# l90lpa/fv3-jedi-linearmodel

Measured on AMD Instinct MI355X. Metric: column-updates/s per TL+AD dyn step, higher is better.
Workload: dtype f64

## Files before the change

fv3_jedi_linearmodel_amd/csrc/fv3lm_capi.cpp:

```cpp
#include "dynamics.h"
#include <array>
#include <string>

using namespace fv3;

struct fv3lm_handle { Dynamics d; };

static thread_local std::string g_err;
static int fail(const std::string& m) { g_err = m; return 1; }
static int g_live = 0;

extern "C" {

const char* fv3lm_last_error(void) { return g_err.c_str(); }

const char* fv3lm_metric_names(void) {
  return "area,rarea,rarea_c,dx,dy,dxa,dya,dxc,dyc,rdx,rdy,rdxa,rdya,rdxc,rdyc,cosa,sina,rsina,cosa_u,cosa_v,cosa_s,"
         "sina_u,sina_v,rsin_u,rsin_v,rsin2,f0,fC,del6_u,del6_v,divg_u,divg_v,"
         "sin_sg1,sin_sg2,sin_sg3,sin_sg4,sin_sg5,sin_sg6,sin_sg7,sin_sg8,sin_sg9,"
         "cos_sg1,cos_sg2,cos_sg3,cos_sg4,cos_sg5,cos_sg6,cos_sg7,cos_sg8,cos_sg9";
}

int fv3lm_create(fv3lm_handle** out, const fv3lm_dims* dm, const fv3lm_options* opt, const double* const* metrics,
                 double da_min, double da_min_c, const double* phis, const double* ak, const double* bk) {
  if (!out || !dm || !opt || !metrics) return fail("fv3lm_create: null argument");
#ifndef FV3LM_HOST_EMUL
  int ndev = 0;
  if (hipGetDeviceCount(&ndev) != hipSuccess || ndev < 1) return fail("fv3lm_create: no HIP device visible (this library has no CPU fallback)");
#endif
  if (!sticky_error().empty()) {
    if (g_live > 0) return fail("fv3lm_create: an earlier failure of a live handle is pending: " + sticky_error());
    sticky_error().clear();
  }
  fv3lm_handle* h = new fv3lm_handle;
  auto bail = [&](std::string e) { h->d.destroy2(); h->d.destroy(); delete h; sticky_error().clear(); return fail("fv3lm_create: " + e); };
  if (!h->d.init(dm->nx, dm->ny, dm->npz, dm->ntile, dm->face, dm->nq, dm->dt, dm->n_split, dm->k_split, *opt, metrics, da_min,
                 da_min_c, phis, dm->nface, dm->tile_ij0)) return bail(h->d.err);
  if (!sticky_error().empty()) return bail(sticky_error());
  if (!h->d.init2(ak, bk)) return bail(h->d.err);
  if (!sticky_error().empty()) return bail(sticky_error());
  *out = h;
  ++g_live;
  return 0;
}

int fv3lm_destroy(fv3lm_handle* h) {
  if (!h) return 0;
  h->d.destroy2(); h->d.destroy(); delete h;
  if (--g_live <= 0) { g_live = 0; sticky_error().clear(); }
  return 0;
}

static bool find(fv3lm_handle* h, const char* name, Fld& f) {
  if (std::string(name) == "phis") { f = Fld{}; f.t = h->d.hs_dev; f.p = h->d.hs_dev; f.nk = 1; return true; }
  auto it = h->d.F.find(name);
  if (it == h->d.F.end()) { g_err = std::string("unknown field ") + name; return false; }
  f = it->second; return true;
}
int fv3lm_field_levels(fv3lm_handle* h, const char* name) { Fld f; return find(h, name, f) ? f.nk : -1; }
int fv3lm_field_put(fv3lm_handle* h, const char* name, int which, const double* host) {
  Fld f; if (!find(h, name, f)) return 1;
  h2d(h->d.ex, which ? f.p : f.t, host, (size_t)h->d.g.ntile * f.nk * h->d.g.plane * 8);
  return sticky_error().empty() ? 0 : fail(sticky_error());
}
int fv3lm_field_get(fv3lm_handle* h, const char* name, int which, double* host) {
  Fld f; if (!find(h, name, f)) return 1;
  d2h(h->d.ex, host, which ? f.p : f.t, (size_t)h->d.g.ntile * f.nk * h->d.g.plane * 8);
  return sticky_error().empty() ? 0 : fail(sticky_error());
}
static int status(fv3lm_handle* h) {
#ifndef FV3LM_HOST_EMUL
  { const hipError_t e = hipGetLastError();
    if (e != hipSuccess) set_sticky(std::string("HIP kernel launch failed: ") + hipGetErrorString(e)); }
  if (const char* dbg = std::getenv("FV3LM_DEBUG_SYNC")) if (dbg[0] == '1') {
    const hipError_t e = hipStreamSynchronize(h->d.ex.stream);
    if (e != hipSuccess) set_sticky(std::string("HIP stream failed: ") + hipGetErrorString(e));
  }
#endif
  if (!sticky_error().empty()) return fail(sticky_error());
  if (!h->d.err.empty() && h->d.halo_missing) return fail(h->d.err);
  if (h->d.halo_missing) return fail("halo exchange needed before fv3lm_set_exchange provided its table (face mode)");
  if (h->d.tracer_subcycle_error) return fail("tracer_2d: accumulated Courant number > 60: trajectory is not usable");
  if (h->d.nh_overflow()) return fail("non-hydrostatic column solver: reverse-mode tape overflow (internal sizing error)");
  return 0;
}
int fv3lm_set_face_data(fv3lm_handle* h, const double* edge, const double* ecorner) {
  if (!edge || !ecorner) return fail("fv3lm_set_face_data: null argument");
  return h->d.set_face_data(edge, ecorner) ? 0 : fail(h->d.err);
}
int fv3lm_set_rayleigh(fv3lm_handle* h, double tau, double rf_cutoff, const double* c2l) {
  if (!h) return fail("fv3lm_set_rayleigh: null handle");
  if (!h->d.set_rayleigh(tau, rf_cutoff, c2l)) return fail(h->d.err);
  return status(h);
}
int fv3lm_rayleigh_profile(fv3lm_handle* h, double* rf, int* kmax) {
  if (!h || !rf || !kmax) return fail("fv3lm_rayleigh_profile: null argument");
  for (int k = 0; k < h->d.g.npz; ++k) rf[k] = k < (int)h->d.rf_host.size() ? h->d.rf_host[(size_t)k] : 0.;
  *kmax = h->d.rf_kmax;
  return 0;
}
int fv3lm_set_exchange(fv3lm_handle* h, int kind, const int* rows, int nrows) {
  if (!rows && nrows > 0) return fail("fv3lm_set_exchange: null table");
  return h->d.set_exchange(kind, rows, nrows) ? 0 : fail(h->d.err);
}
int fv3lm_set_exchange_remote(fv3lm_handle* h, int kind, int npeers, const int* peers, const int* nsend, const int* send_rows, const int* nrecv,
                              const int* recv_rows) {
  return h->d.set_exchange_remote(kind, npeers, peers, nsend, send_rows, nrecv, recv_rows) ? 0 : fail(h->d.err);
}
int fv3lm_comm_unique_id(const char* rccl_path, void* id128) {
#ifndef FV3LM_HOST_EMUL
  std::string e; Transport& T = transport();
  if (!T.load(rccl_path, e)) return fail(e);
  ncclUniqueId id;
  if (T.pGetUniqueId(&id) != ncclSuccess) return fail("ncclGetUniqueId failed");
  std::memcpy(id128, &id, sizeof id);
  return 0;
#else
  (void)rccl_path; (void)id128; return fail("host emulation has no RCCL; use fv3lm_set_transport_callback");
#endif
}
int fv3lm_comm_init(const char* rccl_path, const void* id128, int nranks, int rank) {
#ifndef FV3LM_HOST_EMUL
  std::string e; Transport& T = transport();
  if (!T.load(rccl_path, e)) return fail(e);
  ncclUniqueId id; std::memcpy(&id, id128, sizeof id);
  if (T.pCommInitRank(&T.comm, nranks, id, rank) != ncclSuccess) return fail("ncclCommInitRank failed");
  T.rank = rank; T.nranks = nranks;
  return 0;
#else
  (void)rccl_path; (void)id128; (void)nranks; (void)rank; return fail("host emulation has no RCCL; use fv3lm_set_transport_callback");
#endif
}
int fv3lm_comm_destroy(void) {
#ifndef FV3LM_HOST_EMUL
  Transport& T = transport();
  if (T.comm && T.pCommDestroy) T.pCommDestroy(T.comm);
  T.comm = nullptr;
#endif
  return 0;
}
int fv3lm_set_allreduce_callback(fv3lm_allreduce_fn fn, void* user) { allreduce_max_hook().cb = fn; allreduce_max_hook().user = user; return 0; }
int fv3lm_set_transport_callback(fv3lm_transport_fn fn, void* user) { transport().cb = fn; transport().user = user; return 0; }
int fv3lm_halo(fv3lm_handle* h, int kind, const char* name0, const char* name1, int mode) {
  if (mode < 0 || mode > 2 || kind < 0 || kind >= H_NKIND) return fail("bad mode or kind");
  Fld f0, f1{};
  auto it = h->d.F.find(name0);
  if (it == h->d.F.end()) return fail(std::string("unknown field ") + name0);
  f0 = it->second;
  if (name1 && name1[0]) { it = h->d.F.find(name1); if (it == h->d.F.end()) return fail(std::string("unknown field ") + name1); f1 = it->second; }
  h->d.halo(mode, kind, f0, f1);
  return status(h);
}
int fv3lm_run_group(fv3lm_handle* h, const char* group, int mode) {
  if (mode < 0 || mode > 2) return fail("bad mode");
  h->d.ex.no_wmask = group && group[0];
  h->d.run_group(h->d.acoustic, group, mode);
  h->d.ex.no_wmask = false;
  return status(h);
}
int fv3lm_dyn_core(fv3lm_handle* h, int mode) {
  if (mode < 0 || mode > 2) return fail("bad mode");
  h->d.dyn_core(mode);
  return status(h);
}
int fv3lm_pressures(fv3lm_handle* h, int mode) { h->d.pressures(mode); return status(h); }
int fv3lm_tracer_2d(fv3lm_handle* h, int mode) {
  if (mode == MODE_AD) h->d.tracer_ad(); else h->d.tracer_fwd(mode);
  return status(h);
}
int fv3lm_traj_slots(fv3lm_handle* h) { return (int)h->d.traj_slot.size(); }
int fv3lm_tracer_nsplt(fv3lm_handle* h) { return h->d.nsplt_max; }
int fv3lm_remap(fv3lm_handle* h, int mode, int last_step) { h->d.each_class([&]() { run_remap(h->d.ex, mode, h->d.remap_args(last_step != 0)); }); return status(h); }
int fv3lm_fv_dynamics(fv3lm_handle* h, int mode) { h->d.fv_dynamics(mode); return status(h); }
int fv3lm_rayleigh(fv3lm_handle* h, int mode) {
  if (mode < 0 || mode > 2) return fail("bad mode");
  h->d.rayleigh(mode);
  return status(h);
}
int fv3lm_step_tl(fv3lm_handle* h) { h->d.step_tl(); return status(h); }
int fv3lm_step_nl(fv3lm_handle* h) { h->d.step_nl(); return status(h); }
int fv3lm_step_ad(fv3lm_handle* h) { h->d.step_ad(); return status(h); }
int fv3lm_traj_to_fv3(fv3lm_handle* h, const double* u, const double* v, const double* t, const double* delp, const double* const* q,
                      const double* w, const double* delz, const double* phis) {
  if (!h->d.traj_to_fv3(u, v, t, delp, q, w, delz, phis)) return fail(h->d.err);
  return status(h);
}
int fv3lm_pert_to_fv3(fv3lm_handle* h, const double* u, const double* v, const double* t, const double* delp, const double* const* q,
                      const double* w, const double* delz) {
  if (!h->d.pert_to_fv3(u, v, t, delp, q, w, delz)) return fail(h->d.err);
  return status(h);
}
int fv3lm_fv3_to_pert(fv3lm_handle* h, double* u, double* v, double* t, double* delp, double* const* q, double* w, double* delz) {
  if (!h->d.fv3_to_pert(u, v, t, delp, q, w, delz)) return fail(h->d.err);
  return status(h);
}
int fv3lm_zero_work_adjoint(fv3lm_handle* h) { h->d.zero_work_adjoint(); return 0; }
int fv3lm_sync(fv3lm_handle* h) { dev_sync(h->d.ex); return status(h); }
long fv3lm_launch_count(fv3lm_handle* h) { return h->d.ex.launches; }
int fv3lm_level_params(fv3lm_handle* h, int k, int* ip, double* rp) {
  if (k < 1 || k > h->d.g.npz) return fail("level out of range");
  const LevelParams& l = h->d.lev_host[k - 1];
  ip[0] = l.hord_mt; ip[1] = l.hord_vt; ip[2] = l.hord_tm; ip[3] = l.hord_dp; ip[4] = l.hord_tr;
  ip[5] = l.nord; ip[6] = l.nord_v; ip[7] = l.nord_w; ip[8] = l.nord_t; ip[9] = l.nord_v_pert;
  rp[0] = l.d2_divg; rp[1] = l.damp_vt; rp[2] = l.damp_w; rp[3] = l.damp_t; rp[4] = l.d_con; rp[5] = l.damp_vt_pert;
  return 0;
}
int fv3lm_set_device(int dev) {
#ifndef FV3LM_HOST_EMUL
  if (hipSetDevice(dev) != hipSuccess) return fail("hipSetDevice failed");
#endif
  (void)dev; return 0;
}
int fv3lm_state_save(fv3lm_handle* h) {
  Dynamics& d = h->d; std::vector<Fld> fs{d.f("u"), d.f("v"), d.f("pt"), d.f("delp")};
  if (d.nh) { fs.push_back(d.f("w")); fs.push_back(d.f("delz")); }
  for (auto& q : d.q) fs.push_back(q);
  if (d.snap.size() != fs.size() * 2) { for (double* p : d.snap) dev_free(p); d.snap.clear(); for (size_t n = 0; n < fs.size() * 2; ++n) d.snap.push_back((double*)dev_alloc(d.n3 * 8)); }
  for (size_t n = 0; n < fs.size(); ++n) { dev_copy(d.ex, d.snap[2 * n], fs[n].t, d.n3 * 8); dev_copy(d.ex, d.snap[2 * n + 1], fs[n].p, d.n3 * 8); }
  return 0;
}
int fv3lm_state_restore(fv3lm_handle* h) {
  Dynamics& d = h->d; std::vector<Fld> fs{d.f("u"), d.f("v"), d.f("pt"), d.f("delp")};
  if (d.nh) { fs.push_back(d.f("w")); fs.push_back(d.f("delz")); }
  for (auto& q : d.q) fs.push_back(q);
  if (d.snap.size() != fs.size() * 2) return fail("fv3lm_state_restore: no snapshot");
  for (size_t n = 0; n < fs.size(); ++n) { dev_copy(d.ex, fs[n].t, d.snap[2 * n], d.n3 * 8); dev_copy(d.ex, fs[n].p, d.snap[2 * n + 1], d.n3 * 8); }
  return 0;
}
int fv3lm_profile_begin(fv3lm_handle* h) { h->d.ex.recs.clear(); h->d.ex.profiling = true; return 0; }
int fv3lm_profile_end(fv3lm_handle* h, char* buf, int buflen) {
  Exec& ex = h->d.ex; ex.profiling = false; dev_sync(ex);
  std::map<std::string, std::array<double, 3>> agg;
  for (ProfRec& r : ex.recs) {
    float ms = 0.f;
#ifndef FV3LM_HOST_EMUL
    (void)hipEventElapsedTime(&ms, r.e0, r.e1); (void)hipEventDestroy(r.e0); (void)hipEventDestroy(r.e1);
#endif
    auto& a = agg[r.name]; a[0] += 1.; a[1] += ms; a[2] += r.bytes;
  }
  ex.recs.clear();
  std::string out;
  for (auto& kv : agg) { char line[256]; std::snprintf(line, sizeof line, "%s %.0f %.6f %.0f\n", kv.first.c_str(), kv.second[0], kv.second[1], kv.second[2]); out += line; }
  if (buf && buflen > 0) { std::strncpy(buf, out.c_str(), buflen - 1); buf[buflen - 1] = 0; }
  return (int)out.size() + 1;
}
#ifdef FV3LM_HOST_EMUL
int fv3lm_emul_check_boxes(fv3lm_handle* h, int on) { h->d.ex.check_boxes = on != 0; return 0; }
#endif

}
```

fv3_jedi_linearmodel_amd/csrc/remap.h:

```cpp
#pragma once
#include "column.h"

namespace fv3 {

struct ColWs {
  double* base; size_t stride; int kw;
  HD double& at(int slot, int k) const { return base[((size_t)slot * kw + k) * stride]; }
};
template <class T> struct WsIO;
template <> struct WsIO<double> {
  static constexpr int W = 1;
  HD static double get(const ColWs& w, int s, int k) { return w.at(s, k); }
  HD static void set(const ColWs& w, int s, int k, double x) { w.at(s, k) = x; }
};
template <> struct WsIO<Dual> {
  static constexpr int W = 2;
  HD static Dual get(const ColWs& w, int s, int k) { return Dual(w.at(2 * s, k), w.at(2 * s + 1, k)); }
  HD static void set(const ColWs& w, int s, int k, const Dual& x) { w.at(2 * s, k) = x.v; w.at(2 * s + 1, k) = x.d; }
};

constexpr double R3 = 1. / 3., R23 = 2. / 3.;

template <class T, class FP1, class FQ1, class FP2, class FOut>
HD void map_col(int km, const FP1& pe1, const FQ1& q1, const FP2& pe2, const FOut& out, const ColWs& ws, int SG, int SE) {
  typedef WsIO<T> W;
  T dpa = pe1(2) - pe1(1), dpb = pe1(3) - pe1(2);
  T grat = dpb / dpa;
  T bet = grat * (grat + 0.5);
  T qf = ((grat + grat) * (grat + 1.) * q1(1) + q1(2)) / bet;
  T gam = (1. + grat * (grat + 1.5)) / bet;
  W::set(ws, SE, 1, qf); W::set(ws, SG, 1, gam);
  T d4 = grat, a_prev = q1(1), dp_prev = dpa;
  for (int k = 2; k <= km; ++k) {
    T dpk = pe1(k + 1) - pe1(k);
    T ak_ = q1(k);
    d4 = dp_prev / dpk;
    bet = 2. + d4 + d4 - gam;
    qf = (3. * (a_prev + d4 * ak_) - qf) / bet;
    gam = d4 / bet;
    W::set(ws, SE, k, qf); W::set(ws, SG, k, gam);
    a_prev = ak_; dp_prev = dpk;
  }
  T a_bot = 1. + d4 * (d4 + 1.5);
  T qe = (2. * d4 * (d4 + 1.) * q1(km) + q1(km - 1) - a_bot * qf) / (d4 * (d4 + 0.5) - a_bot * gam);
  W::set(ws, SE, km + 1, qe);
  for (int k = km; k >= 1; --k) {
    qe = W::get(ws, SE, k) - W::get(ws, SG, k) * qe;
    W::set(ws, SE, k, qe);
  }
  int k0 = 1;
  T qsum = T(0.);
  for (int k = 1; k <= km; ++k) {
    const T p2t = pe2(k), p2b = pe2(k + 1);
    int l; bool found = false;
    for (l = k0; l <= km; ++l)
      if (val(p2t) >= val(pe1(l)) && val(p2t) <= val(pe1(l + 1))) { found = true; break; }
    if (found) {
      const T p1l = pe1(l), p1r = pe1(l + 1), dpl = p1r - p1l;
      const T a1 = q1(l), a2 = W::get(ws, SE, l), a3 = W::get(ws, SE, l + 1), a4 = 3. * (2. * a1 - (a2 + a3));
      const T pl = (p2t - p1l) / dpl;
      if (val(p2b) <= val(p1r)) {
        const T pr = (p2b - p1l) / dpl;
        out(k, a2 + 0.5 * (a4 + a3 - a2) * (pr + pl) - a4 * R3 * (pr * (pr + pl) + pl * pl));
        k0 = l;
        continue;
      }
      qsum = (p1r - p2t) * (a2 + 0.5 * (a4 + a3 - a2) * (1. + pl) - a4 * (R3 * (1. + pl * (1. + pl))));
      int m; bool bottom = false;
      for (m = l + 1; m <= km; ++m) {
        if (val(p2b) > val(pe1(m + 1))) qsum = qsum + (pe1(m + 1) - pe1(m)) * q1(m);
        else { bottom = true; break; }
      }
      if (bottom) {
        const T p1m = pe1(m), dpm = pe1(m + 1) - p1m;
        const T b1 = q1(m), b2 = W::get(ws, SE, m), b3 = W::get(ws, SE, m + 1), b4 = 3. * (2. * b1 - (b2 + b3));
        const T dp = p2b - p1m, esl = dp / dpm;
        qsum = qsum + dp * (b2 + 0.5 * esl * (b3 - b2 + b4 * (1. - R23 * esl)));
        k0 = m;
      }
    }
    out(k, qsum / (p2b - p2t));
  }
}

HD void cs_limiters(bool extm, double a1, double& a2, double& a3, double& a4, int iv) {
  if (iv == 0) {
    if (a1 <= 0.) { a2 = a1; a3 = a1; a4 = 0.; }
    else if (fabs(a3 - a2) < -a4) {
      if (a1 + 0.25 * (a3 - a2) * (a3 - a2) / a4 + a4 * (1. / 12.) < 0.) {
        if (a1 < a3 && a1 < a2) { a3 = a1; a2 = a1; a4 = 0.; }
        else if (a3 > a2) { a4 = 3. * (a2 - a1); a3 = a2 - a4; }
        else { a4 = 3. * (a3 - a1); a2 = a3 - a4; }
      }
    }
    return;
  }
  const bool flat = (iv == 1) ? ((a1 - a2) * (a1 - a3) >= 0.) : extm;
  if (flat) { a2 = a1; a3 = a1; a4 = 0.; return; }
  const double da1 = a3 - a2, da2 = da1 * da1, a6da = a4 * da1;
  if (a6da < -da2) { a4 = 3. * (a2 - a1); a3 = a2 - a4; }
  else if (a6da > da2) { a4 = 3. * (a3 - a1); a2 = a3 - a4; }
}
struct LimProfile { int kord, iv; bool scalar; double qmin; };
template <class FA, class FE>
HD void lim_layer(const LimProfile& P, int k, int km, const FA& a1, const FE& qe, double& a2, double& a3, double& a4) {
  const int ak = P.kord < 0 ? -P.kord : P.kord, iv = P.iv;
  auto qlim = [&](int j) -> double {
    double q = qe(j);
    if (j <= 1 || j >= km + 1) return q;
    const double lo = fmin(a1(j - 1), a1(j)), hi = fmax(a1(j - 1), a1(j));
    if (j == 2 || j == km) return fmax(fmin(q, hi), lo);
    const double g1 = a1(j - 1) - a1(j - 2), g2 = a1(j + 1) - a1(j);
    if (g1 * g2 > 0.) return fmax(fmin(q, hi), lo);
    if (g1 > 0.) return fmax(q, lo);
    q = fmin(q, hi);
    return iv == 0 ? fmax(0., q) : q;
  };
  auto gam = [&](int j) { return a1(j) - a1(j - 1); };
  auto extm = [&](int j) -> bool {
    return gam(j) * gam(j + 1) < 0.;
  };
  const double a = a1(k);
  a2 = qlim(k); a3 = qlim(k + 1);
  if (k == 1 || k == km) {
    const bool ex = (a2 - a) * (a3 - a) > 0.;
    if (k == 1) {
      if (iv == 0) a2 = fmax(0., a2);
      else if (iv == -1) { if (a2 * a <= 0.) a2 = 0.; }
    } else {
      if (iv == 0) a3 = fmax(0., a3);
      else if (iv == -1) { if (a3 * a <= 0.) a3 = 0.; }
    }
    a4 = 3. * (2. * a - (a2 + a3));
    cs_limiters(ex, a, a2, a3, a4, 1);
    return;
  }
  if (k == 2 || k == km - 1) { a4 = 3. * (2. * a - (a2 + a3)); cs_limiters(extm(k), a, a2, a3, a4, 2); return; }
  const bool ex = extm(k), small = P.scalar && a < P.qmin;
  auto huynh = [&]() {
    const double pmp_1 = a - 2. * gam(k + 1), lac_1 = pmp_1 + 1.5 * gam(k + 2);
    a2 = fmin(fmax(a2, fmin(a, fmin(pmp_1, lac_1))), fmax(a, fmax(pmp_1, lac_1)));
    const double pmp_2 = a + 2. * gam(k), lac_2 = pmp_2 - 1.5 * gam(k - 1);
    a3 = fmin(fmax(a3, fmin(a, fmin(pmp_2, lac_2))), fmax(a, fmax(pmp_2, lac_2)));
  };
  if (ak == 9) {
    if (ex && (extm(k - 1) || extm(k + 1) || small)) { a2 = a; a3 = a; a4 = 0.; }
    else {
      a4 = 3. * (2. * a - (a2 + a3));
      if (fabs(a4) > fabs(a2 - a3)) { huynh(); a4 = 3. * (2. * a - (a2 + a3)); }
    }
  } else if (ak == 10) {
    if (ex) {
      if (small || extm(k - 1) || extm(k + 1)) { a2 = a; a3 = a; a4 = 0.; }
      else a4 = 6. * a - 3. * (a2 + a3);
    } else {
      a4 = 6. * a - 3. * (a2 + a3);
      if (fabs(a4) > fabs(a2 - a3)) { huynh(); a4 = 6. * a - 3. * (a2 + a3); }
    }
  } else if (ak == 8) {
    huynh(); a4 = 3. * (2. * a - (a2 + a3));
  } else if (ak == 12) {
    if (ex) { a2 = a; a3 = a; a4 = 0.; }
    else {
      a4 = 6. * a - 3. * (a2 + a3);
      if (fabs(a4) > fabs(a2 - a3)) { huynh(); a4 = 6. * a - 3. * (a2 + a3); }
    }
  } else if (ak == 13) {
    if (ex) {
      if (extm(k - 1) && extm(k + 1)) { a2 = a; a3 = a; a4 = 0.; }
      else { huynh(); a4 = 3. * (2. * a - (a2 + a3)); }
    } else a4 = 3. * (2. * a - (a2 + a3));
  } else if (ak == 14) {
    a4 = 3. * (2. * a - (a2 + a3));
  } else {
// ... 525 lines not shown
  typedef RemapAdSlots R_;
  auto pe1 = [&](int k) { return a.pe.t[fidx(g, a.pe, tile, i, j, k)]; };
  auto pn1 = [&](int k) { return a.peln.t[fidx(g, a.peln, tile, i, j, k)]; };
  auto pk1 = [&](int k) { return a.pk.t[fidx(g, a.pk, tile, i, j, k)]; };
  const double ps = pe1(km + 1);
  auto pe2 = [&](int k) -> double { return k == 1 ? a.ptop : (k == km + 1 ? ps : a.ak[k - 1] + a.bk[k - 1] * ps); };
  auto pn2 = [&](int k) -> double { return (k == 1 || k == km + 1) ? pn1(k) : log(pe2(k)); };
  auto pk2 = [&](int k) -> double { return (k == 1 || k == km + 1) ? pk1(k) : exp(a.akap * pn2(k)); };
  auto ptin = [&](int k) { return a.pt.t[fidx(g, a.pt, tile, i, j, k)]; };
  auto tv = [&](int k) -> double { return ptin(k) * (pk1(k + 1) - pk1(k)) / (a.akap * (pn1(k + 1) - pn1(k))); };
  for (int k = 0; k <= km + 1; ++k)
    for (int s_ : {R_::SPE1, R_::SPN1, R_::SPK1, R_::SPE2, R_::SPN2, R_::SPK2}) ws.at(s_, k) = 0.;
  {
    auto outT = [&](int k, double x) { ws.at(R_::ST2, k) = x; };
    bool done = false;
    if constexpr (LIM) if (kord_limited(a.kord_tm)) { map_col_lim(LimProfile{a.kord_tm, 1, true, 184.}, km, pn1, tv, pn2, outT, ws, 0, 1); done = true; }
    if (!done) map_col<double>(km, pn1, tv, pn2, outT, ws, 0, 1);
    if (a.nq > 0 && a.last_step) {
      auto q1 = [&](int k) { return a.q[0].t[fidx(g, a.q[0], tile, i, j, k)]; };
      auto outQ = [&](int k, double x) { ws.at(R_::SQ2, k) = x; };
      bool doneq = false;
      if constexpr (LIM) if (kord_limited(a.kord_tr)) { map_col_lim(LimProfile{a.kord_tr, 0, true, 0.}, km, pe1, q1, pe2, outQ, ws, 0, 1); doneq = true; }
      if (!doneq) map_col<double>(km, pe1, q1, pe2, outQ, ws, 0, 1);
    }
  }
  for (int k = 1; k <= km; ++k) {
    const size_t n0 = fidx(g, a.pt, tile, i, j, k);
    const double pk_hi = pk2(k), pk_lo = pk2(k + 1), pn_hi = pn2(k), pn_lo = pn2(k + 1);
    const double den = a.akap * (pn_lo - pn_hi), pkz = (pk_lo - pk_hi) / den;
    const double pt_ad = a.pt.p[n0], t2 = ws.at(R_::ST2, k);
    double pkz_ad = a.pkz.p[n0], t2_ad;
    if (a.last_step) {
      const double qv = a.nq > 0 ? ws.at(R_::SQ2, k) : 0., f = 1. + a.zvir * qv;
      t2_ad = pt_ad / f;
      if (a.nq > 0) a.q[0].p[fidx(g, a.q[0], tile, i, j, k)] += -(t2 / f) * a.zvir * pt_ad / f;
    } else {
      t2_ad = pt_ad / pkz;
      pkz_ad += -(t2 / pkz) * pt_ad / pkz;
    }
    ws.at(R_::SV, k) = t2_ad;
    const double za = pkz_ad / den;
    ws.at(R_::SPK2, k + 1) += za; ws.at(R_::SPK2, k) -= za;
    const double zb = -pkz * a.akap * za;
    ws.at(R_::SPN2, k + 1) += zb; ws.at(R_::SPN2, k) -= zb;
    const double dpa = a.delp.p[n0];
    ws.at(R_::SPE2, k + 1) += dpa; ws.at(R_::SPE2, k) -= dpa;
    a.delp.p[n0] = 0.; a.pkz.p[n0] = 0.;
  }
  for (int k = 2; k <= km; ++k) {
    ws.at(R_::SPK2, k) += a.pk.p[fidx(g, a.pk, tile, i, j, k)];
    ws.at(R_::SPN2, k) += a.peln.p[fidx(g, a.peln, tile, i, j, k)];
  }
}
HD void remap_ad_k2(const RemapArgs& a, int field, int i, int j, int tile, size_t col) {
  const Geom& g = a.g; const int km = g.npz;
  const ColWs ws{a.ws + col, a.ws_stride, km + 2};
  const FieldAdSlots S = remap_field_slots(field);
  auto pe1 = [&](int k) { return a.pe.t[fidx(g, a.pe, tile, i, j, k)]; };
  const double ps = pe1(km + 1);
  auto pe2 = [&](int k) -> double { return k == 1 ? a.ptop : (k == km + 1 ? ps : a.ak[k - 1] + a.bk[k - 1] * ps); };
  auto p1out = [&](int k, double x) { ws.at(S.SP1, k) = x; };
  auto p2out = [&](int k, double x) { ws.at(S.SP2, k) = x; };
  if (field == 0) {
    auto pn1 = [&](int k) { return a.peln.t[fidx(g, a.peln, tile, i, j, k)]; };
    auto pk1 = [&](int k) { return a.pk.t[fidx(g, a.pk, tile, i, j, k)]; };
    auto pn2 = [&](int k) -> double { return (k == 1 || k == km + 1) ? pn1(k) : log(pe2(k)); };
    auto tv = [&](int k) -> double { return a.pt.t[fidx(g, a.pt, tile, i, j, k)] * (pk1(k + 1) - pk1(k)) / (a.akap * (pn1(k + 1) - pn1(k))); };
    auto q2ad = [&](int k) { return ws.at(RemapAdSlots::SV, k); };
    map_col_ad_s(km, pn1, tv, pn2, q2ad, ws, S.w, [&](int k, double x) { ws.at(S.SQ1, k) = x; }, p1out, p2out);
  } else {
    const Fld& qf = a.q[field - 1];
    auto q1 = [&](int k) { return qf.t[fidx(g, qf, tile, i, j, k)]; };
    auto q2ad = [&](int k) { return qf.p[fidx(g, qf, tile, i, j, k)]; };
    map_col_ad_s(km, pe1, q1, pe2, q2ad, ws, S.w, [&](int k, double x) { qf.p[fidx(g, qf, tile, i, j, k)] = x; }, p1out, p2out);
  }
}
HD void remap_ad_k3(const RemapArgs& a, int i, int j, int tile, size_t col) {
  const Geom& g = a.g; const int km = g.npz;
  const ColWs ws{a.ws + col, a.ws_stride, km + 2};
  typedef RemapAdSlots R_;
  auto pe1 = [&](int k) { return a.pe.t[fidx(g, a.pe, tile, i, j, k)]; };
  auto pn1 = [&](int k) { return a.peln.t[fidx(g, a.peln, tile, i, j, k)]; };
  auto pk1 = [&](int k) { return a.pk.t[fidx(g, a.pk, tile, i, j, k)]; };
  const double ps = pe1(km + 1);
  auto pe2 = [&](int k) -> double { return k == 1 ? a.ptop : (k == km + 1 ? ps : a.ak[k - 1] + a.bk[k - 1] * ps); };
  auto pn2 = [&](int k) -> double { return (k == 1 || k == km + 1) ? pn1(k) : log(pe2(k)); };
  auto pk2 = [&](int k) -> double { return (k == 1 || k == km + 1) ? pk1(k) : exp(a.akap * pn2(k)); };
  {
    const FieldAdSlots S = remap_field_slots(0);
    for (int k = 1; k <= km + 1; ++k) { ws.at(R_::SPN1, k) += ws.at(S.SP1, k); ws.at(R_::SPN2, k) += ws.at(S.SP2, k); }
    for (int k = 1; k <= km; ++k) {
      const double tv_ad = ws.at(S.SQ1, k), dpk = pk1(k + 1) - pk1(k), den = a.akap * (pn1(k + 1) - pn1(k)), pt0 = a.pt.t[fidx(g, a.pt, tile, i, j, k)];
      a.pt.p[fidx(g, a.pt, tile, i, j, k)] = tv_ad * dpk / den;
      const double za = pt0 * tv_ad / den;
      ws.at(R_::SPK1, k + 1) += za; ws.at(R_::SPK1, k) -= za;
      const double zb = -(pt0 * dpk / den) * a.akap * tv_ad / den;
      ws.at(R_::SPN1, k + 1) += zb; ws.at(R_::SPN1, k) -= zb;
    }
  }
  for (int n = 0; n < a.nq; ++n) {
    const FieldAdSlots S = remap_field_slots(1 + n);
    for (int k = 1; k <= km + 1; ++k) { ws.at(R_::SPE1, k) += ws.at(S.SP1, k); ws.at(R_::SPE2, k) += ws.at(S.SP2, k); }
  }
  for (int k = 2; k <= km; ++k) {
    const double pn_ad = ws.at(R_::SPN2, k) + a.akap * pk2(k) * ws.at(R_::SPK2, k);
    ws.at(R_::SPE2, k) += pn_ad / pe2(k);
  }
  for (int k : {1, km + 1}) {
    ws.at(R_::SPN1, k) += ws.at(R_::SPN2, k) + a.peln.p[fidx(g, a.peln, tile, i, j, k)];
    ws.at(R_::SPK1, k) += ws.at(R_::SPK2, k) + a.pk.p[fidx(g, a.pk, tile, i, j, k)];
  }
  double ps_ad = ws.at(R_::SPE2, km + 1);
  for (int k = 2; k <= km; ++k) ps_ad += a.bk[k - 1] * ws.at(R_::SPE2, k);
  ws.at(R_::SPE1, km + 1) += ps_ad;
  for (int k = 1; k <= km + 1; ++k) {
    a.pk.p[fidx(g, a.pk, tile, i, j, k)] = ws.at(R_::SPK1, k);
    a.peln.p[fidx(g, a.peln, tile, i, j, k)] = ws.at(R_::SPN1, k);
    a.pe.p[fidx(g, a.pe, tile, i, j, k)] += ws.at(R_::SPE1, k);
  }
}

template <int MODE, bool LIM = false>
struct RemapFieldFn {
  RemapArgs a; int nf;
  HD void operator()(int i, int j, int z) const {
    const int tile = z / nf, field = z % nf;
    const size_t col = (size_t)tile * a.g.plane + a.g.idx(i, j);
    if (MODE == MODE_NL) remap_field_col<double, LIM>(a, field, i, j, tile, col);
    else if (MODE == MODE_TL) remap_field_col<Dual, LIM>(a, field, i, j, tile, col);
    else remap_ad_k2(a, field, i, j, tile, col);
  }
};
template <int MODE, bool LIM = false>
struct RemapPressFn {
  RemapArgs a;
  HD void operator()(int i, int j, int z) const {
    const size_t col = (size_t)z * a.g.plane + a.g.idx(i, j);
    if (MODE == MODE_NL) remap_press_col<double>(a, i, j, z);
    else if (MODE == MODE_TL) remap_press_col<Dual>(a, i, j, z);
    else if (MODE == MODE_AD) remap_ad_k1<LIM>(a, i, j, z, col);
    else remap_ad_k3(a, i, j, z, col);
  }
};
template <int MODE, bool LIM = false>
struct RemapWindFn {
  RemapArgs a; int dir;
  HD void operator()(int i, int j, int z) const {
    const size_t col = (size_t)z * a.g.plane + a.g.idx(i, j);
    if (MODE == MODE_NL) remap_wind_col<double, LIM>(a, dir, i, j, z, col);
    else if (MODE == MODE_TL) remap_wind_col<Dual, LIM>(a, dir, i, j, z, col);
    else remap_wind_col_ad(a, dir, i, j, z, col);
  }
};
inline void run_remap_winds(Exec& ex, int mode, const RemapArgs& a, double bytes = 0.) {
  const Geom& g = a.g;
  const Rect U{g.is(), g.ie(), g.js(), g.je() + 1}, V{g.is(), g.ie() + 1, g.js(), g.je()};
  if (kord_limited(a.kord_mt) && mode != MODE_AD) {
    if (mode == MODE_NL) { for_points(ex, U, g.ntile, RemapWindFn<MODE_NL, true>{a, 0}, "remap_wind_lim.nl", bytes); for_points(ex, V, g.ntile, RemapWindFn<MODE_NL, true>{a, 1}, "remap_wind_lim.nl", bytes); }
    else { for_points(ex, U, g.ntile, RemapWindFn<MODE_TL, true>{a, 0}, "remap_wind_lim.tl", bytes); for_points(ex, V, g.ntile, RemapWindFn<MODE_TL, true>{a, 1}, "remap_wind_lim.tl", bytes); }
  }
  else if (mode == MODE_NL) { for_points(ex, U, g.ntile, RemapWindFn<MODE_NL>{a, 0}, "remap_wind.nl", bytes); for_points(ex, V, g.ntile, RemapWindFn<MODE_NL>{a, 1}, "remap_wind.nl", bytes); }
  else if (mode == MODE_TL) { for_points(ex, U, g.ntile, RemapWindFn<MODE_TL>{a, 0}, "remap_wind.tl", bytes); for_points(ex, V, g.ntile, RemapWindFn<MODE_TL>{a, 1}, "remap_wind.tl", bytes); }
  else { for_points(ex, V, g.ntile, RemapWindFn<MODE_AD>{a, 1}, "remap_wind.ad", bytes); for_points(ex, U, g.ntile, RemapWindFn<MODE_AD>{a, 0}, "remap_wind.ad", bytes); }
}
struct RemapGatherFn {
  RemapArgs a;
  HD void operator()(int i, int j, int z) const { remap_pe_gather_ad(a, i, j, z); }
};
struct RemapPeFn {
  RemapArgs a; int mode;
  HD void operator()(int i, int j, int z) const {
    for (int k = 2; k <= a.g.npz; ++k) {
      const size_t n = fidx(a.g, a.pe, z, i, j, k);
      a.pe.t[n] = a.pe2.t[n];
      if (mode == MODE_TL) a.pe.p[n] = a.pe2.p[n];
    }
  }
};

inline int remap_ws_slots(int nq) { return RemapAdSlots::FBASE + RemapAdSlots::FN * (1 + nq); }
inline void run_remap(Exec& ex, int mode, const RemapArgs& a) {
  const Geom& g = a.g;
  const Rect A{g.is(), g.ie(), g.js(), g.je()}, H{g.is() - 1, g.ie() + 1, g.js() - 1, g.je() + 1};
  if (mode != MODE_AD) {
    const double cells = double(g.tx) * g.ty * g.ntile * g.npz, w = mode == MODE_TL ? 2. : 1.;
    const int nf = 1 + a.nq;
    const bool lim = kord_limited(a.kord_tm) || kord_limited(a.kord_tr);
    if (lim && mode == MODE_TL) {
      for_points(ex, A, g.ntile * nf, RemapFieldFn<MODE_TL, true>{a, nf}, "remap_fields_lim.tl", 8. * w * (5. + 2. * a.nq) * cells);
      for_points(ex, A, g.ntile, RemapPressFn<MODE_TL>{a}, "remap_press.tl", 8. * w * (5. + 7.) * cells);
    } else if (lim) {
      for_points(ex, A, g.ntile * nf, RemapFieldFn<MODE_NL, true>{a, nf}, "remap_fields_lim.nl", 8. * w * (5. + 2. * a.nq) * cells);
      for_points(ex, A, g.ntile, RemapPressFn<MODE_NL>{a}, "remap_press.nl", 8. * w * (5. + 7.) * cells);
    } else if (mode == MODE_TL) {
      for_points(ex, A, g.ntile * nf, RemapFieldFn<MODE_TL>{a, nf}, "remap_fields.tl", 8. * w * (5. + 2. * a.nq) * cells);
      for_points(ex, A, g.ntile, RemapPressFn<MODE_TL>{a}, "remap_press.tl", 8. * w * (5. + 7.) * cells);
    } else {
      for_points(ex, A, g.ntile * nf, RemapFieldFn<MODE_NL>{a, nf}, "remap_fields.nl", 8. * w * (5. + 2. * a.nq) * cells);
      for_points(ex, A, g.ntile, RemapPressFn<MODE_NL>{a}, "remap_press.nl", 8. * w * (5. + 7.) * cells);
    }
    run_remap_winds(ex, mode, a, 8. * w * 4. * cells);
    for_points(ex, A, g.ntile, RemapPeFn{a, mode}, "remap_pe");
  } else {
    const double cells = double(g.tx) * g.ty * g.ntile * g.npz;
    run_remap_winds(ex, MODE_AD, a, 8. * 7. * cells);
    for_points(ex, H, g.ntile, RemapGatherFn{a}, "remap_gather.ad", 8. * 4. * cells);
    const int nf = 1 + a.nq;
    if (kord_limited(a.kord_tm) || kord_limited(a.kord_tr)) for_points(ex, A, g.ntile, RemapPressFn<MODE_AD, true>{a}, "remap_scalars1_lim.ad", 8. * 12. * cells);
    else for_points(ex, A, g.ntile, RemapPressFn<MODE_AD>{a}, "remap_scalars1.ad", 8. * 12. * cells);
    for_points(ex, A, g.ntile * nf, RemapFieldFn<MODE_AD>{a, nf}, "remap_fields.ad", 8. * (4. + 3. * a.nq) * cells);
    for_points(ex, A, g.ntile, RemapPressFn<3>{a}, "remap_scalars3.ad", 8. * 8. * cells);
  }
}

}
```

Measured before the change: 186,900.

## Parallelize vertical remap tridiagonal solve across wavefront lanes with associative scans

Adds wave-level parallel remap kernels for the NL/TL field and wind remaps. The sequential tridiagonal recurrences of the PPM edge solve become Möbius and affine compositions combined with a 64-lane shuffle scan, and columns are staged in LDS. The goal is to remove the serial per-column vertical loop that leaves threads underused. In exchange it adds LDS pressure and extra arithmetic, changes floating-point association (rescaled Möbius products), and keeps an environment variable fallback to the sequential path.

```diff
diff --git a/fv3_jedi_linearmodel_amd/csrc/colscan.h b/fv3_jedi_linearmodel_amd/csrc/colscan.h
--- /dev/null
+++ b/fv3_jedi_linearmodel_amd/csrc/colscan.h
@@ -0,0 +1,125 @@
+#pragma once
+#include "core.h"
+
+namespace fv3 {
+
+constexpr double R3 = 1. / 3., R23 = 2. / 3.;
+
+template <class T> struct Mob { T a, b, c, d; };
+template <class T> struct Aff { T a, b; };
+template <class T> HD Mob<T> mob_id() { return Mob<T>{T(1.), T(0.), T(0.), T(1.)}; }
+template <class T> HD Aff<T> aff_id() { return Aff<T>{T(1.), T(0.)}; }
+HD double scale2(double x, int e) { return ldexp(x, e); }
+HD Dual scale2(const Dual& x, int e) { return Dual(ldexp(x.v, e), ldexp(x.d, e)); }
+template <class T> HD Mob<T> compose(const Mob<T>& f, const Mob<T>& g) {
+  const T a = g.a * f.a + g.b * f.c, b = g.a * f.b + g.b * f.d, c = g.c * f.a + g.d * f.c, d = g.c * f.b + g.d * f.d;
+  const double m = fmax(fmax(fabs(val(a)), fabs(val(b))), fmax(fabs(val(c)), fabs(val(d))));
+  if (!(m > 0.) || !(m < 1e300)) return Mob<T>{a, b, c, d};
+  const int e = -ilogb(m);
+  return Mob<T>{scale2(a, e), scale2(b, e), scale2(c, e), scale2(d, e)};
+}
+template <class T> HD Aff<T> compose(const Aff<T>& f, const Aff<T>& g) { return Aff<T>{g.a * f.a, g.a * f.b + g.b}; }
+template <class T> HD T chain_value(const Mob<T>& m) { return m.b / m.d; }
+template <class T> HD T chain_value(const Aff<T>& m) { return m.b; }
+
+template <class T> struct ColSolve {
+  int km, P;
+  const T *X, *Q;
+  T *G, *E;
+  HD T x(int k) const { return X[k - 1]; }
+  HD T q(int k) const { return Q[k - 1]; }
+  HD int lo(int lane) const { return lane * P + 1; }
+  HD int hi(int lane, int top) const { const int h = lane * P + P; return h < top ? h : top; }
+  HD T d4(int k) const { return (x(k) - x(k - 1)) / (x(k + 1) - x(k)); }
+  HD T grat() const { return (x(3) - x(2)) / (x(2) - x(1)); }
+};
+
+template <class T> HD Mob<T> gam_local(const ColSolve<T>& s, int lane) {
+  Mob<T> m = mob_id<T>();
+  for (int k = s.lo(lane); k <= s.hi(lane, s.km); ++k) {
+    if (k == 1) { const T gr = s.grat(), bet = gr * (gr + 0.5); m = Mob<T>{T(0.), (1. + gr * (gr + 1.5)) / bet, T(0.), T(1.)}; }
+    else { const T d4 = s.d4(k); m = compose(m, Mob<T>{T(0.), d4, T(-1.), 2. + d4 + d4}); }
+  }
+  return m;
+}
+template <class T> HD void gam_apply(const ColSolve<T>& s, int lane, const Mob<T>& in) {
+  const int k0 = s.lo(lane), k1 = s.hi(lane, s.km);
+  if (k0 > k1) return;
+  T gam = k0 > 1 ? chain_value(in) : T(0.);
+  for (int k = k0; k <= k1; ++k) {
+    if (k == 1) { const T gr = s.grat(), bet = gr * (gr + 0.5); gam = (1. + gr * (gr + 1.5)) / bet; }
+    else { const T d4 = s.d4(k), bet = 2. + d4 + d4 - gam; gam = d4 / bet; }
+    s.G[k - 1] = gam;
+  }
+}
+template <class T> HD Aff<T> qf_local(const ColSolve<T>& s, int lane) {
+  Aff<T> m = aff_id<T>();
+  for (int k = s.lo(lane); k <= s.hi(lane, s.km); ++k) {
+    if (k == 1) { const T gr = s.grat(), bet = gr * (gr + 0.5); m = Aff<T>{T(0.), ((gr + gr) * (gr + 1.) * s.q(1) + s.q(2)) / bet}; }
+    else { const T d4 = s.d4(k), bet = 2. + d4 + d4 - s.G[k - 2]; m = compose(m, Aff<T>{-1. / bet, 3. * (s.q(k - 1) + d4 * s.q(k)) / bet}); }
+  }
+  return m;
+}
+template <class T> HD void qf_apply(const ColSolve<T>& s, int lane, const Aff<T>& in) {
+  const int k0 = s.lo(lane), k1 = s.hi(lane, s.km);
+  if (k0 > k1) return;
+  T qf = k0 > 1 ? chain_value(in) : T(0.);
+  for (int k = k0; k <= k1; ++k) {
+    if (k == 1) { const T gr = s.grat(), bet = gr * (gr + 0.5); qf = ((gr + gr) * (gr + 1.) * s.q(1) + s.q(2)) / bet; }
+    else { const T d4 = s.d4(k), bet = 2. + d4 + d4 - s.G[k - 2]; qf = (3. * (s.q(k - 1) + d4 * s.q(k)) - qf) / bet; }
+    s.E[k - 1] = qf;
+  }
+}
+template <class T> HD T qe_bottom(const ColSolve<T>& s) {
+  const int km = s.km;
+  const T d4 = s.d4(km), a_bot = 1. + d4 * (d4 + 1.5);
+  return (2. * d4 * (d4 + 1.) * s.q(km) + s.q(km - 1) - a_bot * s.E[km - 1]) / (d4 * (d4 + 0.5) - a_bot * s.G[km - 1]);
+}
+template <class T> HD Aff<T> back_local(const ColSolve<T>& s, int lane, const T& qbot) {
+  Aff<T> m = aff_id<T>();
+  for (int k = s.hi(lane, s.km + 1); k >= s.lo(lane); --k)
+    m = k == s.km + 1 ? Aff<T>{T(0.), qbot} : compose(m, Aff<T>{-s.G[k - 1], s.E[k - 1]});
+  return m;
+}
+template <class T> HD void back_apply(const ColSolve<T>& s, int lane, const Aff<T>& in, const T& qbot) {
+  const int k0 = s.lo(lane), k1 = s.hi(lane, s.km + 1);
+  if (k0 > k1) return;
+  T qe = k1 <= s.km ? chain_value(in) : T(0.);
+  for (int k = k1; k >= k0; --k) {
+    qe = k == s.km + 1 ? qbot : s.E[k - 1] - s.G[k - 1] * qe;
+    s.E[k - 1] = qe;
+  }
+}
+
+template <class T> HD T map_target(const ColSolve<T>& s, const T* Y, int k) {
+  const T* E = s.E;
+  const int km = s.km;
+  const T p2t = Y[k - 1], p2b = Y[k];
+  const double vt = val(p2t);
+  int lo = 1, hi = km + 1;
+  while (lo < hi) { const int mid = (lo + hi) >> 1; if (val(s.x(mid + 1)) >= vt) hi = mid; else lo = mid + 1; }
+  const int l = lo;
+  if (!(l <= km && val(s.x(l)) <= vt)) return T(0.);
+  const T p1l = s.x(l), p1r = s.x(l + 1), dpl = p1r - p1l;
+  const T a1 = s.q(l), a2 = E[l - 1], a3 = E[l], a4 = 3. * (2. * a1 - (a2 + a3));
+  const T pl = (p2t - p1l) / dpl;
+  if (val(p2b) <= val(p1r)) {
+    const T pr = (p2b - p1l) / dpl;
+    return a2 + 0.5 * (a4 + a3 - a2) * (pr + pl) - a4 * R3 * (pr * (pr + pl) + pl * pl);
+  }
+  T qsum = (p1r - p2t) * (a2 + 0.5 * (a4 + a3 - a2) * (1. + pl) - a4 * (R3 * (1. + pl * (1. + pl))));
+  int m;
+  for (m = l + 1; m <= km; ++m) {
+    if (val(p2b) > val(s.x(m + 1))) qsum = qsum + (s.x(m + 1) - s.x(m)) * s.q(m);
+    else break;
+  }
+  if (m <= km) {
+    const T p1m = s.x(m), dpm = s.x(m + 1) - p1m;
+    const T b1 = s.q(m), b2 = E[m - 1], b3 = E[m], b4 = 3. * (2. * b1 - (b2 + b3));
+    const T dp = p2b - p1m, esl = dp / dpm;
+    qsum = qsum + dp * (b2 + 0.5 * esl * (b3 - b2 + b4 * (1. - R23 * esl)));
+  }
+  return qsum / (p2b - p2t);
+}
+
+}
diff --git a/fv3_jedi_linearmodel_amd/csrc/fv3lm_capi.cpp b/fv3_jedi_linearmodel_amd/csrc/fv3lm_capi.cpp
--- a/fv3_jedi_linearmodel_amd/csrc/fv3lm_capi.cpp
+++ b/fv3_jedi_linearmodel_amd/csrc/fv3lm_capi.cpp
@@ -1,6 +1,7 @@
 #include "dynamics.h"
 #include <array>
 #include <string>
+#include <vector>
 
 using namespace fv3;
 
@@ -246,6 +247,39 @@
 }
 #ifdef FV3LM_HOST_EMUL
 int fv3lm_emul_check_boxes(fv3lm_handle* h, int on) { h->d.ex.check_boxes = on != 0; return 0; }
-#endif
-
-}
+int fv3lm_emul_col_map(int km, int lanes, const double* pe1, const double* q1, const double* pe2, double* qe_seq, double* out_seq,
+                       double* qe_lanes, double* out_lanes) {
+  if (km < 3 || lanes < 1) return fail("fv3lm_emul_col_map: km >= 3, lanes >= 1");
+  std::vector<double> ws(2 * (km + 2));
+  const ColWs cw{ws.data(), 1, km + 2};
+  map_col<double>(km, [&](int k) { return pe1[k - 1]; }, [&](int k) { return q1[k - 1]; }, [&](int k) { return pe2[k - 1]; },
+                  [&](int k, double x) { out_seq[k - 1] = x; }, cw, 0, 1);
+  for (int k = 1; k <= km + 1; ++k) qe_seq[k - 1] = cw.at(1, k);
+  std::vector<double> G(km + 1);
+  const ColSolve<double> s{km, (km + lanes) / lanes, pe1, q1, G.data(), qe_lanes};
+  auto scan = [&](auto local, auto id, bool rev) {
+    std::vector<decltype(id)> v(lanes), o(lanes);
+    for (int L = 0; L < lanes; ++L) v[L] = local(L);
+    for (int d = 1; d < lanes; d <<= 1) {
+      o = v;
+      for (int L = 0; L < lanes; ++L) {
+        if (!rev && L >= d) v[L] = compose(o[L - d], o[L]);
+        if (rev && L + d < lanes) v[L] = compose(o[L + d], o[L]);
+      }
+    }
+    for (int L = 0; L < lanes; ++L) o[L] = rev ? (L == lanes - 1 ? id : v[L + 1]) : (L == 0 ? id : v[L - 1]);
+    return o;
+  };
+  const auto mg = scan([&](int L) { return gam_local(s, L); }, mob_id<double>(), false);
+  for (int L = 0; L < lanes; ++L) gam_apply(s, L, mg[L]);
+  const auto mf = scan([&](int L) { return qf_local(s, L); }, aff_id<double>(), false);
+  for (int L = 0; L < lanes; ++L) qf_apply(s, L, mf[L]);
+  const double qb = qe_bottom(s);
+  const auto mb = scan([&](int L) { return back_local(s, L, qb); }, aff_id<double>(), true);
+  for (int L = 0; L < lanes; ++L) back_apply(s, L, mb[L], qb);
+  for (int k = 1; k <= km; ++k) out_lanes[k - 1] = map_target(s, pe2, k);
+  return 0;
+}
+#endif
+
+}
diff --git a/fv3_jedi_linearmodel_amd/csrc/remap.h b/fv3_jedi_linearmodel_amd/csrc/remap.h
--- a/fv3_jedi_linearmodel_amd/csrc/remap.h
+++ b/fv3_jedi_linearmodel_amd/csrc/remap.h
@@ -1,5 +1,6 @@
 #pragma once
 #include "column.h"
+#include "colscan.h"
 
 namespace fv3 {
 
@@ -18,8 +19,6 @@
   HD static Dual get(const ColWs& w, int s, int k) { return Dual(w.at(2 * s, k), w.at(2 * s + 1, k)); }
   HD static void set(const ColWs& w, int s, int k, const Dual& x) { w.at(2 * s, k) = x.v; w.at(2 * s + 1, k) = x.d; }
 };
-
-constexpr double R3 = 1. / 3., R23 = 2. / 3.;
 
 template <class T, class FP1, class FQ1, class FP2, class FOut>
 HD void map_col(int km, const FP1& pe1, const FQ1& q1, const FP2& pe2, const FOut& out, const ColWs& ws, int SG, int SE) {
@@ -851,9 +850,171 @@
     else remap_wind_col_ad(a, dir, i, j, z, col);
   }
 };
+inline bool remap_seq() { const char* e = std::getenv("FV3LM_REMAP_SEQ"); return e && e[0] == '1'; }
+struct RemapLanesCfg { int rc, nw; size_t lds; };
+inline bool remap_lanes_cfg(int npz, size_t tsz, RemapLanesCfg& c) {
+  static const int opt[][2] = {{4, 4}, {4, 2}, {2, 2}, {2, 1}, {1, 1}};
+  for (const auto& o : opt) {
+    c.rc = o[0]; c.nw = o[1]; c.lds = (size_t)(2 * o[0] + 3 * o[1]) * (npz + 1) * tsz;
+    if (c.lds <= 160 * 1024) return true;
+  }
+  return false;
+}
+#ifndef FV3LM_HOST_EMUL
+DEV void wave_sync() { __builtin_amdgcn_fence(__ATOMIC_RELEASE, "workgroup"); __builtin_amdgcn_wave_barrier(); __builtin_amdgcn_fence(__ATOMIC_ACQUIRE, "workgroup"); }
+DEV double lane_up(double x, int d) { return __shfl_up(x, d); }
+DEV double lane_down(double x, int d) { return __shfl_down(x, d); }
+DEV Dual lane_up(const Dual& x, int d) { return Dual(__shfl_up(x.v, d), __shfl_up(x.d, d)); }
+DEV Dual lane_down(const Dual& x, int d) { return Dual(__shfl_down(x.v, d), __shfl_down(x.d, d)); }
+template <class T> DEV Mob<T> lane_up(const Mob<T>& m, int d) { return Mob<T>{lane_up(m.a, d), lane_up(m.b, d), lane_up(m.c, d), lane_up(m.d, d)}; }
+template <class T> DEV Aff<T> lane_up(const Aff<T>& m, int d) { return Aff<T>{lane_up(m.a, d), lane_up(m.b, d)}; }
+template <class T> DEV Aff<T> lane_down(const Aff<T>& m, int d) { return Aff<T>{lane_down(m.a, d), lane_down(m.b, d)}; }
+template <class M> DEV M wave_excl(M agg, int lane, const M& id) {
+  for (int d = 1; d < 64; d <<= 1) { const M o = lane_up(agg, d); if (lane >= d) agg = compose(o, agg); }
+  const M e = lane_up(agg, 1);
+  return lane == 0 ? id : e;
+}
+template <class M> DEV M wave_excl_rev(M agg, int lane, const M& id) {
+  for (int d = 1; d < 64; d <<= 1) { const M o = lane_down(agg, d); if (lane + d < 64) agg = compose(o, agg); }
+  const M e = lane_down(agg, 1);
+  return lane == 63 ? id : e;
+}
+template <class T>
+DEV void map_col_wave(int km, const T* X, T* Q, const T* Y, T* G, T* E, int lane) {
+  const ColSolve<T> s{km, (km + 64) / 64, X, Q, G, E};
+  gam_apply(s, lane, wave_excl(gam_local(s, lane), lane, mob_id<T>()));
+  wave_sync();
+  qf_apply(s, lane, wave_excl(qf_local(s, lane), lane, aff_id<T>()));
+  wave_sync();
+  const T qb = qe_bottom(s);
+  back_apply(s, lane, wave_excl_rev(back_local(s, lane, qb), lane, aff_id<T>()), qb);
+  wave_sync();
+  for (int k = s.lo(lane); k <= s.hi(lane, km); ++k) G[k - 1] = map_target(s, Y, k);
+  wave_sync();
+  for (int k = s.lo(lane); k <= s.hi(lane, km); ++k) Q[k - 1] = G[k - 1];
+}
+template <class T>
+__global__ void __launch_bounds__(512) k_remap_fields_lanes(RemapArgs a, int RC) {
+  extern __shared__ __attribute__((aligned(16))) unsigned char rl_lds[];
+  typedef FIO<T> IO;
+  const Geom& g = a.g; const int km = g.npz, S = km + 1;
+  int bx = blockIdx.x, by = blockIdx.y; xcd_block(gridDim.x, gridDim.y, bx, by);
+  const int i0 = g.is() + bx * RC, j = g.js() + by, tile = blockIdx.z, nc = min(RC, g.ie() - i0 + 1);
+  const int t = threadIdx.x, nt = blockDim.x, w = t >> 6, lane = t & 63, nw = nt >> 6;
+  T* Xs = reinterpret_cast<T*>(rl_lds); T* Qs = Xs + RC * S;
+  T* Y = Qs + RC * S + 3 * S * w; T* G = Y + S; T* E = G + S;
+  auto at = [&](const Fld& f, int c, int k) { return fidx(g, f, tile, i0 + c, j, k); };
+  auto store = [&](const Fld& f) {
+    for (int e = t; e < RC * km; e += nt) { const int c = e % RC, k = e / RC + 1; if (c < nc) IO::st(f, at(f, c, k), Qs[c * S + k - 1]); }
+  };
+  for (int e = t; e < RC * S; e += nt) { const int c = e % RC, k = e / RC + 1; if (c < nc) Xs[c * S + k - 1] = IO::ld(a.peln, at(a.peln, c, k)); }
+  __syncthreads();
+  for (int e = t; e < RC * km; e += nt) {
+    const int c = e % RC, k = e / RC + 1;
+    if (c < nc) Qs[c * S + k - 1] = IO::ld(a.pt, at(a.pt, c, k)) * (IO::ld(a.pk, at(a.pk, c, k + 1)) - IO::ld(a.pk, at(a.pk, c, k))) /
+                                    (a.akap * (Xs[c * S + k] - Xs[c * S + k - 1]));
+  }
+  __syncthreads();
+  for (int c = w; c < nc; c += nw) {
+    const T ps = IO::ld(a.pe, at(a.pe, c, km + 1));
+    for (int k = lane + 1; k <= S; k += 64) Y[k - 1] = (k == 1 || k == S) ? Xs[c * S + k - 1] : dlog(a.ak[k - 1] + a.bk[k - 1] * ps);
+    wave_sync();
+    map_col_wave(km, Xs + c * S, Qs + c * S, Y, G, E, lane);
+    wave_sync();
+  }
+  __syncthreads();
+  store(a.pt);
+  if (a.nq == 0) return;
+  __syncthreads();
+  for (int e = t; e < RC * S; e += nt) { const int c = e % RC, k = e / RC + 1; if (c < nc) Xs[c * S + k - 1] = IO::ld(a.pe, at(a.pe, c, k)); }
+  for (int n = 0; n < a.nq; ++n) {
+    const Fld& qf = a.q[n];
+    for (int e = t; e < RC * km; e += nt) { const int c = e % RC, k = e / RC + 1; if (c < nc) Qs[c * S + k - 1] = IO::ld(qf, at(qf, c, k)); }
+    __syncthreads();
+    for (int c = w; c < nc; c += nw) {
+      const T ps = Xs[c * S + km];
+      for (int k = lane + 1; k <= S; k += 64) Y[k - 1] = k == 1 ? T(a.ptop) : (k == S ? ps : a.ak[k - 1] + a.bk[k - 1] * ps);
+      wave_sync();
+      map_col_wave(km, Xs + c * S, Qs + c * S, Y, G, E, lane);
+      wave_sync();
+    }
+    __syncthreads();
+    store(qf);
+    __syncthreads();
+  }
+}
+template <class T>
+__global__ void __launch_bounds__(512) k_remap_wind_lanes(RemapArgs a, int RC, int dir, Rect R) {
+  extern __shared__ __attribute__((aligned(16))) unsigned char rl_lds[];
+  typedef FIO<T> IO;
+  const Geom& g = a.g; const int km = g.npz, S = km + 1;
+  int bx = blockIdx.x, by = blockIdx.y; xcd_block(gridDim.x, gridDim.y, bx, by);
+  const int i0 = R.i0 + bx * RC, j = R.j0 + by, tile = blockIdx.z, nc = min(RC, R.i1 - i0 + 1);
+  const int t = threadIdx.x, nt = blockDim.x, w = t >> 6, lane = t & 63, nw = nt >> 6;
+  const int di = dir == 0 ? 0 : -1, dj = dir == 0 ? -1 : 0;
+  const Fld& wf = dir == 0 ? a.u : a.v;
+  T* Xs = reinterpret_cast<T*>(rl_lds); T* Qs = Xs + RC * S;
+  T* Y = Qs + RC * S + 3 * S * w; T* G = Y + S; T* E = G + S;
+  for (int e = t; e < RC * S; e += nt) {
+    const int c = e % RC, k = e / RC + 1, i = i0 + c;
+    if (c >= nc) continue;
+    Xs[c * S + k - 1] = k == 1 ? IO::ld(a.pe, fidx(g, a.pe, tile, i, j, 1))
+                               : 0.5 * (IO::ld(a.pe, fidx(g, a.pe, tile, i + di, j + dj, k)) + IO::ld(a.pe, fidx(g, a.pe, tile, i, j, k)));
+    if (k <= km) Qs[c * S + k - 1] = IO::ld(wf, fidx(g, wf, tile, i, j, k));
+  }
+  __syncthreads();
+  for (int c = w; c < nc; c += nw) {
+    const int i = i0 + c;
+    const T pss = IO::ld(a.pe, fidx(g, a.pe, tile, i + di, j + dj, km + 1)) + IO::ld(a.pe, fidx(g, a.pe, tile, i, j, km + 1));
+    for (int k = lane + 1; k <= S; k += 64) Y[k - 1] = (dir == 1 && k == 1) ? T(a.ak[0]) : a.ak[k - 1] + (0.5 * a.bk[k - 1]) * pss;
+    wave_sync();
+    map_col_wave(km, Xs + c * S, Qs + c * S, Y, G, E, lane);
+    wave_sync();
+  }
+  __syncthreads();
+  for (int e = t; e < RC * km; e += nt) { const int c = e % RC, k = e / RC + 1; if (c < nc) IO::st(wf, fidx(g, wf, tile, i0 + c, j, k), Qs[c * S + k - 1]); }
+}
+inline bool remap_lanes_prep(const void* kfn, bool& attr, RemapLanesCfg& cf, int npz, size_t tsz) {
+  if (!remap_lanes_cfg(npz, tsz, cf)) return false;
+  if (!attr) {
+    if (hipFuncSetAttribute(kfn, hipFuncAttributeMaxDynamicSharedMemorySize, 160 * 1024) != hipSuccess) set_sticky("hipFuncSetAttribute(remap lanes) failed");
+    attr = true;
+  }
+  return true;
+}
+template <class T>
+bool run_remap_fields_lanes(Exec& ex, const RemapArgs& a, const char* tag, double bytes) {
+  const Geom& g = a.g; RemapLanesCfg cf; static bool attr = false;
+  if (!remap_lanes_prep((const void*)k_remap_fields_lanes<T>, attr, cf, g.npz, sizeof(T))) return false;
+  ex.mark_begin(tag, "", bytes);
+  hipLaunchKernelGGL(k_remap_fields_lanes<T>, dim3((g.tx + cf.rc - 1) / cf.rc, g.ty, g.ntile), dim3(64 * cf.nw), cf.lds, ex.stream, a, cf.rc);
+  ex.mark_end();
+  ex.launches++;
+  return true;
+}
+template <class T>
+bool run_remap_wind_lanes(Exec& ex, const RemapArgs& a, int dir, const Rect& R, const char* tag, double bytes) {
+  const Geom& g = a.g; RemapLanesCfg cf; static bool attr = false;
+  if (!remap_lanes_prep((const void*)k_remap_wind_lanes<T>, attr, cf, g.npz, sizeof(T))) return false;
+  ex.mark_begin(tag, "", bytes);
+  hipLaunchKernelGGL(k_remap_wind_lanes<T>, dim3((R.i1 - R.i0 + cf.rc) / cf.rc, R.j1 - R.j0 + 1, g.ntile), dim3(64 * cf.nw), cf.lds, ex.stream, a, cf.rc, dir, R);
+  ex.mark_end();
+  ex.launches++;
+  return true;
+}
+#else
+template <class T> bool run_remap_fields_lanes(Exec&, const RemapArgs&, const char*, double) { return false; }
+template <class T> bool run_remap_wind_lanes(Exec&, const RemapArgs&, int, const Rect&, const char*, double) { return false; }
+#endif
+
 inline void run_remap_winds(Exec& ex, int mode, const RemapArgs& a, double bytes = 0.) {
   const Geom& g = a.g;
   const Rect U{g.is(), g.ie(), g.js(), g.je() + 1}, V{g.is(), g.ie() + 1, g.js(), g.je()};
+  if (!kord_limited(a.kord_mt) && mode != MODE_AD && !remap_seq()) {
+    const bool ok = mode == MODE_NL ? run_remap_wind_lanes<double>(ex, a, 0, U, "remap_wind.nl", bytes) && run_remap_wind_lanes<double>(ex, a, 1, V, "remap_wind.nl", bytes)
+                                    : run_remap_wind_lanes<Dual>(ex, a, 0, U, "remap_wind.tl", bytes) && run_remap_wind_lanes<Dual>(ex, a, 1, V, "remap_wind.tl", bytes);
+    if (ok) return;
+  }
   if (kord_limited(a.kord_mt) && mode != MODE_AD) {
     if (mode == MODE_NL) { for_points(ex, U, g.ntile, RemapWindFn<MODE_NL, true>{a, 0}, "remap_wind_lim.nl", bytes); for_points(ex, V, g.ntile, RemapWindFn<MODE_NL, true>{a, 1}, "remap_wind_lim.nl", bytes); }
     else { for_points(ex, U, g.ntile, RemapWindFn<MODE_TL, true>{a, 0}, "remap_wind_lim.tl", bytes); for_points(ex, V, g.ntile, RemapWindFn<MODE_TL, true>{a, 1}, "remap_wind_lim.tl", bytes); }
@@ -892,10 +1053,12 @@
       for_points(ex, A, g.ntile * nf, RemapFieldFn<MODE_NL, true>{a, nf}, "remap_fields_lim.nl", 8. * w * (5. + 2. * a.nq) * cells);
       for_points(ex, A, g.ntile, RemapPressFn<MODE_NL>{a}, "remap_press.nl", 8. * w * (5. + 7.) * cells);
     } else if (mode == MODE_TL) {
-      for_points(ex, A, g.ntile * nf, RemapFieldFn<MODE_TL>{a, nf}, "remap_fields.tl", 8. * w * (5. + 2. * a.nq) * cells);
+      if (remap_seq() || !run_remap_fields_lanes<Dual>(ex, a, "remap_fields.tl", 8. * w * (5. + 2. * a.nq) * cells))
+        for_points(ex, A, g.ntile * nf, RemapFieldFn<MODE_TL>{a, nf}, "remap_fields.tl", 8. * w * (5. + 2. * a.nq) * cells);
       for_points(ex, A, g.ntile, RemapPressFn<MODE_TL>{a}, "remap_press.tl", 8. * w * (5. + 7.) * cells);
     } else {
-      for_points(ex, A, g.ntile * nf, RemapFieldFn<MODE_NL>{a, nf}, "remap_fields.nl", 8. * w * (5. + 2. * a.nq) * cells);
+      if (remap_seq() || !run_remap_fields_lanes<double>(ex, a, "remap_fields.nl", 8. * w * (5. + 2. * a.nq) * cells))
+        for_points(ex, A, g.ntile * nf, RemapFieldFn<MODE_NL>{a, nf}, "remap_fields.nl", 8. * w * (5. + 2. * a.nq) * cells);
       for_points(ex, A, g.ntile, RemapPressFn<MODE_NL>{a}, "remap_press.nl", 8. * w * (5. + 7.) * cells);
     }
     run_remap_winds(ex, mode, a, 8. * w * 4. * cells);
```

New measurement: 188,500, median of 6. About the same (+0.8%).
